# medvedevgroup/TwoPaCo

Measured on AMD Instinct MI355X. Metric: kmers_hashed_per_sec, higher is better.
Workload: dtype u64

## Files before the change

### twopaco_amd/csrc/tpc_capi.hip

```cpp
#include "tpc_ctx.h"

namespace tpch {

int fail(tpc_ctx *c, int code, const char *fmt, ...)
{
    char buf[512];
    va_list ap;
    va_start(ap, fmt);
    vsnprintf(buf, sizeof buf, fmt, ap);
    va_end(ap);
    if (c) c->err = buf;
    return code;
}





TpcLaunch make_launch(const tpc_ctx *c)
{
    TpcLaunch a;
    a.P = c->P; a.tab = c->tab; a.bases = c->bases; a.nmask = c->nmask; a.n_text = c->n_text;
    a.n_tiles = c->n_tiles; a.filter = c->filter; a.stream = c->stream;
    a.stat_kernel = c->stat_kernel;
// ... 175 lines not shown
bool replicated(const tpc_ctx *c) { return c->opt_replicate && c->sh_world > 1; }
void pass_tiles(const tpc_ctx *c, uint64_t &t_begin, uint64_t &t_end)
{
    const uint64_t tiles = text_tiles512(c);
    t_begin = 0; t_end = tiles;
    if (replicated(c)) {
        const uint64_t chunk = (tiles + c->sh_world - 1) / c->sh_world;
        t_begin = std::min<uint64_t>(tiles, (uint64_t)c->sh_rank * chunk);
        t_end = std::min<uint64_t>(tiles, t_begin + chunk);
    }
}
uint64_t pass_tile_count(const tpc_ctx *c) { uint64_t a, b; pass_tiles(c, a, b); return std::max<uint64_t>(1, b - a); }

size_t qpart_need(const TpcQPlan &pl, int i)
{
    if (i == 0) return std::max(tpc_qpart_bytes(pl, 0), tpc_qpart_bytes(pl, 9));
    if (i == 9) return 0;
    return tpc_qpart_bytes(pl, i);
}

bool part_hash_supported(const tpc_ctx *c)
{
    if (c->P.q > TPC_KERNEL_MAXQ || tpc_test_force_anyq) return false;
    if (c->P.q > 8 && (c->P.L - c->opt_slice_bits > 24 || c->no_lean)) return false;
    return true;
}

bool plan_query(const tpc_ctx *c, uint64_t lo, uint64_t hi, bool gated, TpcQPlan &pl)
{
    const uint64_t tiles = pass_tile_count(c);
    if (c->P.q > TPC_KERNEL_MAXQ || tpc_test_force_anyq) return false;
// ... 87 lines not shown
}

const char *tpc_last_error(const tpc_ctx *c) { return c ? c->err.c_str() : "null context"; }

int tpc_set_option(tpc_ctx *c, const char *name, int64_t value)
{
    if (!c || !name) return -1;
    if (!strcmp(name, "insert_test_first")) { c->opt_test_first = value != 0; return 0; }
    if (!strcmp(name, "insert_mode")) { c->opt_insert_mode = (int)value; return 0; }
    if (!strcmp(name, "slice_bits")) { c->opt_slice_bits = (int)value; return 0; }
    if (!strcmp(name, "query_mode")) { c->opt_query_mode = (int)value; return 0; }
    if (!strcmp(name, "part_budget_bytes")) { c->opt_part_budget = value; return 0; }
    if (!strcmp(name, "part_levels")) { c->opt_part_levels = (int)value; return 0; }
    if (!strcmp(name, "shard_tight_regions")) { c->opt_shard_tight = value ? 1 : 0; c->sh_have[0] = c->sh_have[1] = false; return 0; }
    if (!strcmp(name, "part_min_tiles")) { c->opt_part_min_tiles = value < 1 ? 1 : value; return 0; }
    if (!strcmp(name, "fuse_apply_lookup")) { c->opt_fuse = value != 0; return 0; }
    if (!strcmp(name, "test_q6_pb2")) { tpc_test_q6_pb2 = (int)value; return 0; }
    if (!strcmp(name, "insert_entry_fmt")) { tpc_test_insert_p3 = value == 3; return 0; }
    if (!strcmp(name, "shard_periodic_skip")) { c->opt_shard_periodic = value != 0; return 0; }
    if (!strcmp(name, "periodic_skip")) { c->opt_periodic = value != 0; if (!value) c->periodic_valid = false; return 0; }
    if (!strcmp(name, "test_tight_pinch")) { tpc_test_tight_pinch = (int)value; c->sh_have[0] = c->sh_have[1] = false; return 0; }
    if (!strcmp(name, "test_sched_cap")) { tpc_test_sched_cap = value > 0 ? (uint32_t)value : 0; return 0; }
    if (!strcmp(name, "text_window")) { c->opt_text_window = value != 0; return 0; }
    if (!strcmp(name, "replicate_filter")) { c->opt_replicate = value != 0; return 0; }
    if (!strcmp(name, "test_force_anyq")) { tpc_test_force_anyq = value != 0; return 0; }
    if (!strcmp(name, "test_sketch_grid")) { tpc_test_sketch_grid = value > 0 ? (int)value : 0; return 0; }
    if (!strcmp(name, "test_links_slots_log2")) { c->opt_links_slots_log2 = (int)std::max<int64_t>(-1, std::min<int64_t>(value, 64)); return 0; }
    if (!strcmp(name, "test_distances_chunk_words")) { c->opt_distances_chunk_words = (int)std::max<int64_t>(-1, std::min<int64_t>(value, 1 << 20)); return 0; }
    if (!strcmp(name, "test_fail_mallocs")) { tpc_test_fail_mallocs.store(value > 0 ? (int)value : 0); return 0; }
    return fail(c, -1, "unknown option %s", name);
// ... 17 lines not shown
{
    if (!c) return -1;
    return tpc_preload(c->device);
}

int64_t tpc_get_stat(const tpc_ctx *c, const char *name)
{
    if (!c || !name) return -1;
    if (!strcmp(name, "insert_path")) return c->stat_path[0];
    if (!strcmp(name, "query_path")) return c->stat_path[1];
    if (!strcmp(name, "insert_entry_fmt")) return c->stat_fmt[0];
    if (!strcmp(name, "query_entry_fmt")) return c->stat_fmt[1];
    if (!strcmp(name, "insert_hash_kernel")) return c->stat_kernel[0];
    if (!strcmp(name, "query_hash_kernel")) return c->stat_kernel[1];
    if (!strcmp(name, "query_verify_kernel")) return c->stat_kernel[2];
    if (!strcmp(name, "insert_batches")) return c->stat_batches[0];
    if (!strcmp(name, "query_batches")) return c->stat_batches[1];
    if (!strcmp(name, "query_tiles_per_batch")) return c->stat_q_plan[0];
    if (!strcmp(name, "query_b1")) return c->stat_q_plan[1];
    if (!strcmp(name, "query_b2")) return c->stat_q_plan[2];
    if (!strcmp(name, "query_begun")) return c->stat_q_begun;
    if (!strcmp(name, "filter2_retries")) return c->stat_filter2_retries;
    if (!strcmp(name, "aggregate_retries")) return c->stat_aggregate_retries;
    if (!strcmp(name, "filter2_counted")) return c->stat_filter2_counted;
    if (!strcmp(name, "fused_lookups")) return c->stat_fused;
    if (!strcmp(name, "query_overflow_entries")) return c->stat_query_overflow;
    if (!strcmp(name, "insert_overflow_entries")) return c->stat_insert_overflow;
    if (!strcmp(name, "periodic_skip")) return c->periodic_valid ? 1 : 0;
    if (!strcmp(name, "pbuf_releases")) return c->stat_pbuf_releases;
    if (!strcmp(name, "distances_tile")) return TPC_DISTANCES_TILE;
// ... 404 lines not shown
    if (part)
        for (int i = 0; i < tpc_ctx::NPBUF && part; i++) if (qpart_need(pl, i)) part = ensure_pbuf(c, i, qpart_need(pl, i));
    const bool fused = !begin_only && part && fuses(pl);
    if (!fused && !begin_only) { int rc0 = materialize_reset(c); if (rc0) return rc0; }
    if (part) {
        pl.buf1 = (uint64_t *)c->pbuf[0]; pl.cnt1 = (uint32_t *)c->pbuf[1]; pl.buf2 = (uint64_t *)c->pbuf[2]; pl.cnt2 = (uint32_t *)c->pbuf[3];
        pl.ovf = (uint64_t *)c->pbuf[4]; pl.ovf_cur = (unsigned long long *)c->pbuf[5];
        pl.surv = (uint64_t *)c->pbuf[6]; pl.surv_cur = (unsigned long long *)c->pbuf[7];
        pl.off2 = (const uint64_t *)c->pbuf[8];
        if (c->off2_uploaded != pl.off2_host) {
            HIPCHK(c, hipMemcpy(c->pbuf[8], pl.off2_host.data(), pl.off2_host.size() * 8, hipMemcpyHostToDevice));
            c->off2_uploaded = pl.off2_host;
        }
        pl.buf3 = (uint64_t *)c->pbuf[0]; pl.cnt3 = (uint32_t *)c->pbuf[10]; pl.off3 = (const uint64_t *)c->pbuf[11];
        pl.bnd = (uint32_t *)c->pbuf[18];
        if (pl.b3 && c->off3_uploaded != pl.off3_host) {
            HIPCHK(c, hipMemcpy(c->pbuf[11], pl.off3_host.data(), pl.off3_host.size() * 8, hipMemcpyHostToDevice));
            c->off3_uploaded = pl.off3_host;
        }
        unsigned long long f1[2] = {0, 0}, f2 = 0;
        bool overflowed = false;
        uint64_t per_batch = 1;
        {
            Timed t(c, TPC_K_QUERY);
            const uint64_t per = pl.n_tiles;
            per_batch = per;
            for (uint64_t t0 = t_begin; (t0 < t_end || t0 == t_begin) && !overflowed; t0 += per) {
                pl.tile0 = t0;
                pl.tile0_global = t0;
                pl.n_tiles = t0 < t_end ? std::min<uint64_t>(per, t_end - t0) : 0;
                const bool presplit = begun && t0 == t_begin;
                if (!presplit) {
                    HIPCHK(c, hipMemsetAsync(pl.ovf_cur, 0, 32 * sizeof(unsigned long long), c->stream));
                    HIPCHK(c, hipMemsetAsync(pl.surv_cur, 0, TPC_SURV_CUR_WORDS * sizeof(unsigned long long), c->stream));
                }
                if (begin_only) {
                    TpcQPlan p1 = pl;
                    p1.rbuf1 = p1.buf1; p1.rcnt1 = p1.cnt1;
                    if (tpc_launch_query_part_hash(make_launch_periodic(c), p1, c->rmask, lo, hi, gated) || tpc_launch_query_part_split(make_launch(c), p1))
                        return fail(c, -1, "partitioned query launch failed");
                    HIPCHK(c, hipGetLastError());
                    c->qb_valid = true; c->qb_lo = lo; c->qb_hi = hi;
// ... 22 lines not shown
                    p1.rbuf1 = p1.buf1; p1.rcnt1 = p1.cnt1;
                    p1.presplit = true;
                    if (tpc_launch_query_part_lookup(make_launch(c), p1) || tpc_launch_query_verify(make_launch(c), p1, c->rmask)) return fail(c, -1, "partitioned query launch failed");
                } else
                if (tpc_launch_query_partitioned(make_launch_periodic(c), pl, c->rmask, lo, hi, gated)) return fail(c, -1, "partitioned query launch failed");
                HIPCHK(c, hipMemcpyAsync(f1, pl.ovf_cur, sizeof f1, hipMemcpyDeviceToHost, c->stream));
                HIPCHK(c, hipMemcpyAsync(&f2, pl.surv_cur + 64, sizeof f2, hipMemcpyDeviceToHost, c->stream));
                if (t0 + per < t_end) {
                    unsigned long long sc[TPC_SURV_CUR_WORDS], batch_marks = 0;
                    const uint64_t w0 = t0 * 512, wn = std::min<uint64_t>(pl.n_tiles * 512, c->n_words > w0 ? c->n_words - w0 : 0);
                    if (wn) tpc_launch_mask_count(c->stream, c->rmask + w0, wn, c->block_sums, c->counters + 3);
                    HIPCHK(c, hipMemcpyAsync(sc, pl.surv_cur, sizeof sc, hipMemcpyDeviceToHost, c->stream));
                    if (wn) HIPCHK(c, hipMemcpyAsync(&batch_marks, c->counters + 3, sizeof batch_marks, hipMemcpyDeviceToHost, c->stream));
                    HIPCHK(c, hipStreamSynchronize(c->stream));
                    overflowed = f1[1] != 0 || f2 != 0;
                    unsigned long long surv = 0;
                    for (int i = 0; i < 64; i++) surv += std::min<unsigned long long>(sc[i], pl.surv_cap);
                    if (surv > 0) pl.group_survivors = batch_marks * 4 >= surv;
                }
            }
            if (c->periodic_valid && c->periodic_any_q && c->periodic) tpc_launch_periodic_copy(c->stream, c->rmask, c->periodic, c->periodic + c->n_words_alloc, c->n_words_alloc, c->n_words);
            tpc_launch_mask_count(c->stream, c->rmask, c->n_words, c->block_sums, c->counters + 1);
        }
        HIPCHK(c, hipGetLastError());
        uint64_t n = 0;
        int rc = read_counter(c, 1, &n);
        if (rc) return rc;
        overflowed = overflowed || f1[1] != 0 || f2 != 0;
        c->stat_query_overflow = (int64_t)f1[0];
        c->stat_path[1] = (pl.b3 ? 3 : 2) + (overflowed ? 10 : 0);
        c->stat_fmt[1] = pl.fmt;
        c->stat_batches[1] = (int64_t)((pass_tile_count(c) + per_batch - 1) / per_batch);
        c->stat_q_plan[0] = (int64_t)per_batch; c->stat_q_plan[1] = pl.b1; c->stat_q_plan[2] = pl.b2;
        if (c->dbg_ovf) {
            unsigned long long sc[65];
            (void)hipMemcpy(sc, pl.surv_cur, sizeof sc, hipMemcpyDeviceToHost);
            unsigned long long tot = 0, most = 0;
            for (int i = 0; i < 64; i++) { tot += sc[i]; most = std::max(most, sc[i]); }
            fprintf(stderr, "[ovf] query: %llu overflow entries (cap %llu, flag %llu), survivors %llu (fullest list %llu of %llu, flag %llu) b1=%d b2=%d ppr=%d loads=%d\n", f1[0],
                    (unsigned long long)pl.ovf_cap, f1[1], tot, most, (unsigned long long)pl.surv_cap, f2, pl.b1, pl.b2, pl.pos_per_round, pl.loads);
            static const char *const dump_path = getenv("TPC_DUMP_SURV");
            if (const char *path = dump_path) {
                if (FILE *fp = fopen(path, "w")) {
                    for (int i = 0; i < 64; i++) {
                        const size_t n = (size_t)std::min<unsigned long long>(sc[i], pl.surv_cap);
// ... 42 lines not shown
        }
        if (c->dbg_phases) {
            unsigned long long pr[32];
            (void)hipMemcpy(pr, pl.ovf_cur, sizeof pr, hipMemcpyDeviceToHost);
            fprintf(stderr, "[phases] ovf=%llu  split: push %llu book %llu copy %llu rounds %llu | hash: push %llu book %llu copy %llu rounds %llu (10 ns ticks summed over WGs) | lost at level 1: %llu, at level 2/3: %llu\n",
                    pr[0], pr[8], pr[9], pr[10], pr[12], pr[16], pr[17], pr[18], pr[20], pr[25], pr[27]);
        }
        if (!overflowed) {
            c->rmask_sums_valid = true;
            c->rmask_sums_n = n;
            if (n_marks) *n_marks = n;
            return 0;
        }
        if (replicated(c)) return fail(c, -20, "overflow or survivor list overflowed (address skew beyond what the sharded path handles)");
    }
    if (!part) { c->stat_path[1] = 1; c->stat_batches[1] = 1; }
    HIPCHK(c, hipMemsetAsync(c->counters + 1, 0, sizeof(unsigned long long), c->stream));
    {
        Timed t(c, TPC_K_QUERY);
        TpcLaunch ad = make_launch(c);
        if (replicated(c)) { ad.g_begin = t_begin * 512ull * TPC_RUN; ad.g_end = t_end * 512ull * TPC_RUN; }
        if (part) ad.stat_kernel = nullptr;
        if (tpc_launch_query(ad, c->rmask, lo, hi, gated, c->counters + 1)) return fail(c, -1, "query launch failed");
    }
    HIPCHK(c, hipGetLastError());
    uint64_t n = 0;
    int rc = read_counter(c, 1, &n);
    if (rc) return rc;
    if (n_marks) *n_marks = n;
    return 0;
}
// ... 83 lines not shown
```

### twopaco_amd/csrc/tpc_ctx.h

```cpp
#pragma once
#include "../../include/twopaco_hip.h"
#include "tpc_internal.h"

#include <algorithm>
#include <atomic>
#include <cmath>
#include <chrono>
#include <cstdarg>
#include <cstdio>
#include <cstdlib>
#include <cstring>
#include <string>
#include <vector>
#include <map>

struct tpc_ctx {
    int device = 0;
    hipStream_t stream = nullptr;
    std::string err;
    bool have_params = false;
    TpcHashParams P{};
    uint64_t tab_host[TPC_TAB_WORDS]{};
    uint64_t *tab = nullptr;
    int C = 1;
// ... 90 lines not shown
    int opt_slice_bits = 20;
    bool filter_zero_pending = false;
    static constexpr int NPBUF = 19;
    void *pbuf[NPBUF] = {};
    size_t pbytes[NPBUF] = {};
    std::vector<uint64_t> off2_uploaded, off3_uploaded;
    int opt_part_levels = 0;
    int opt_shard_tight = 1;
    int stat_path[2] = {0, 0};
    int64_t stat_batches[2] = {0, 0};
    mutable int stat_kernel[3] = {0, 0, 0};
    int stat_fmt[2] = {0, 0};
    int64_t stat_filter2_retries = 0;
    int64_t stat_aggregate_retries = 0;
    int stat_filter2_counted = 0;
    int64_t opt_part_min_tiles = 256;
    int64_t opt_part_budget = 0;
    int opt_query_mode = 0;
    int opt_fuse = 1;
    bool pending_apply = false;
    bool pending_fresh = false;
    bool pending_shard = false;
    TpcPartPlan pending_pl;
    void *ikeep[2] = {nullptr, nullptr};
    size_t ikeep_bytes[2] = {0, 0};
    uint64_t *ikeep_ovf = nullptr;
    uint64_t ikeep_ovf_cap = 0;
    uint64_t pending_novf = 0;
    uint32_t *iovf_cnt = nullptr;
    uint64_t *iovf_off = nullptr;
// ... 97 lines not shown
```

### twopaco_amd/csrc/tpc_internal.h

```cpp
#pragma once
#include "tpc_device.h"
#include <algorithm>
#include <cstdlib>
#include <vector>

struct TpcEnv {
    bool no_lean, rb_hash, verify_eager, gated_full;
    int ppr_insert, gated_loads, split_loads9;
    int slice_grid;
    static const TpcEnv &get()
    {
        static const TpcEnv e = [] {
            TpcEnv v;
            v.no_lean = getenv("TPC_NO_LEAN") != nullptr;
            v.rb_hash = getenv("TPC_RB_HASH") != nullptr;
            const char *lz = getenv("TPC_VERIFY_LAZY");
            v.verify_eager = lz && lz[0] == '0';
            v.gated_full = getenv("TPC_GATED_FULL_REGIONS") != nullptr;
            const char *p = getenv("TPC_PPR_INSERT"), *g = getenv("TPC_GATED_LOADS");
            v.ppr_insert = p ? atoi(p) : 0;
            v.gated_loads = g ? atoi(g) : 0;
            const char *s9 = getenv("TPC_SPLIT_LOADS9");
            v.split_loads9 = s9 ? atoi(s9) : 0;
            const char *lg = getenv("TPC_LOOKUP_GRID");
            int n_cu = 0, dev = 0;
            if (hipGetDevice(&dev) != hipSuccess || hipDeviceGetAttribute(&n_cu, hipDeviceAttributeMultiprocessorCount, dev) != hipSuccess || n_cu <= 0) { (void)hipGetLastError(); n_cu = 256; }
            v.slice_grid = lg ? atoi(lg) : 2 * n_cu;
            return v;
        }();
        return e;
    }
};

// ... 97 lines not shown
    uint64_t *ovf;
    unsigned long long *ovf_cur;
    uint64_t *surv;
    unsigned long long *surv_cur;
    uint32_t rank = 0, world = 1;
    const uint64_t *rbuf1 = nullptr;
    const uint32_t *rcnt1 = nullptr;
    const uint64_t *roff1 = nullptr;
    const uint64_t *rown1 = nullptr;
    const uint32_t *rowncnt1 = nullptr;
    bool group_survivors = true;
    int fmt = 0;
    bool presplit = false;
    uint32_t tiles_per_wg = 0, n_groups = 0, pb2 = 0;
    uint32_t *bnd = nullptr;
};
#define TPC_SURV_CUR_WORDS 72
bool tpc_qpart_plan(int L, int slice_bits, uint64_t n_tiles, double frac, TpcQPlan &pl, int levels = 0);
size_t tpc_qpart_bytes(const TpcQPlan &pl, int which);
bool tpc_qpart_plan_sharded(int L, int slice_bits, uint64_t n_tiles, double frac, uint32_t rank, uint32_t world, TpcQPlan &pl, int levels = 0, bool tight = false,
                            bool packed = false);
int tpc_launch_query_partitioned(const TpcLaunch &a, const TpcQPlan &pl, uint32_t *rmask, uint64_t lo, uint64_t hi, bool gated);
int tpc_launch_insert_part_split(const TpcLaunch &a, const TpcPartPlan &pl);
int tpc_launch_insert_part_apply_only(const TpcLaunch &a, const TpcPartPlan &pl, bool fresh);
struct TpcListSrc;
int tpc_launch_query_part_fused_lookup(const TpcLaunch &a, const TpcQPlan &pl, const TpcPartPlan &ipl, bool fresh, const uint64_t *iovf_sorted, const uint64_t *iovf_off,
                                       const TpcListSrc *lists = nullptr);
int tpc_launch_ovf_by_slice(const TpcLaunch &a, const uint64_t *list, uint64_t n, int slice_bits, uint32_t n_slices, uint32_t *cnt, uint32_t *cursor,
                            uint64_t *off, uint64_t *sorted, uint32_t rank = 0, uint32_t world = 1, int log_nb2 = 0);
#define TPC_FUSE_MAX_OVF (16ull << 20)
int tpc_launch_query_verify(const TpcLaunch &a, const TpcQPlan &pl, uint32_t *rmask);
extern int tpc_test_tight_pinch;
extern int tpc_test_q6_pb2;
extern int tpc_test_insert_p3;
extern uint32_t tpc_test_sched_cap;
int tpc_launch_region_offsets(const TpcLaunch &a, const uint32_t *cnt, uint32_t n_regions, uint64_t *off);
int tpc_launch_region_pack(const TpcLaunch &a, const void *regions, uint64_t cap_entries, uint32_t entry_bytes, const uint32_t *cnt, const uint64_t *off,
                           uint32_t n_regions, void *packed);
int tpc_launch_query_part_hash(const TpcLaunch &a, const TpcQPlan &pl, uint32_t *rmask, uint64_t lo, uint64_t hi, bool gated);
int tpc_launch_query_part_lookup(const TpcLaunch &a, const TpcQPlan &pl);
int tpc_launch_query_part_split(const TpcLaunch &a, const TpcQPlan &pl);
int tpc_launch_surv_gather(const TpcLaunch &a, const TpcQPlan &pl, uint64_t *out);
int tpc_launch_verify_addrs(const TpcLaunch &a, const TpcQPlan &pl, int fn, int fn_count, const uint64_t *sid, uint64_t n, uint64_t *addr_out, int32_t *owner_out,
                            unsigned long long *owner_counts = nullptr);
#define TPC_V_OWNER_SHIFT 56
int tpc_launch_finish(hipStream_t s, const TpcQPlan &pl, const uint64_t *sid, uint64_t n, int fn_count, const uint8_t *hit, const uint32_t *perm, uint32_t *rmask,
                      unsigned long long *n_marked);
// ... 103 lines not shown
```

### twopaco_amd/csrc/tpc_qpartition.hip

```cpp
#ifndef TPC_QPARTITION_PART
#define TPC_QPARTITION_PART 0
#endif
#include "tpc_rbins.h"
#include "tpc_bins3.h"
#include "tpc_binsp.h"
#include "tpc_lean.h"
#include "tpc_internal.h"
#include "tpc_lists.h"
#include <algorithm>
#include <type_traits>
#include <cstdio>
#include <cstdlib>
#include <cmath>

#if TPC_QPARTITION_PART == 0
int tpc_test_q6_pb2 = 0;
#endif

namespace {

constexpr int QE_E_SHIFT = 31;
constexpr uint64_t QE_REM_MASK = (1ull << QE_E_SHIFT) - 1ull;
constexpr int QS_LISTS = 64;

struct QOverflow {
    uint64_t *list;
    unsigned long long *cursor;
    uint64_t cap;
    __device__ __forceinline__ void push(uint64_t addr, uint64_t sid, int site = 0) const
    {
#ifdef TPC_PROFILE_PHASES
// ... 725 lines not shown
        if (hit) {
            const uint32_t lane = threadIdx.x & 63u, leader = (uint32_t)__ffsll((long long)m) - 1u;
            unsigned long long base = 0;
            if (lane == leader) base = atomicAdd(&surv_cur[0], (unsigned long long)__popcll(m));
            base = __shfl(base, (int)leader, 64);
            const unsigned long long o = base + (unsigned long long)__popcll(m & ((1ull << lane) - 1ull));
            if (o < surv_cap) surv[o] = list[2 * i + 1]; else surv_cur[QS_LISTS] = 1ull;
        }
    }
}

#endif
template <int Q>
__global__ void __launch_bounds__(256)
k_q_verify(TpcHashParams P, const uint64_t *__restrict__ tab, const uint64_t *__restrict__ bases, const uint32_t *__restrict__ filter,
           const uint64_t *__restrict__ surv, const unsigned long long *__restrict__ surv_cur, uint64_t surv_cap, uint64_t gbase, uint32_t *rmask)
{
    __shared__ uint64_t s_h[Q * 5], s_hk[Q * 5];
    if (threadIdx.x < Q * 5) { s_h[threadIdx.x] = tab[threadIdx.x]; s_hk[threadIdx.x] = tab[TPC_TAB_HK + threadIdx.x]; }
    __syncthreads();
    const int list = blockIdx.y;
    const uint64_t n = min((uint64_t)surv_cur[list], surv_cap);
    const uint64_t *my = surv + (uint64_t)list * surv_cap;
    const uint64_t stride = (uint64_t)gridDim.x * blockDim.x;
    for (uint64_t idx = (uint64_t)blockIdx.x * blockDim.x + threadIdx.x; idx < n; idx += stride) {
        const uint64_t sid = my[idx];
        if (sid == ~0ull) continue;
        const int e = (int)(sid & 7);
        const uint64_t g = gbase + (sid >> 3);
        const int c = e & 3;
        auto roll = [&](auto lo_tag, auto hi_tag, bool neg_strand, uint64_t (&h)[Q]) {
            constexpr int LO = decltype(lo_tag)::value, HI = decltype(hi_tag)::value;
#pragma unroll
            for (int i = LO; i < HI; i++) h[i] = 0;
            if (!neg_strand) {
                for (int t0 = 0; t0 < P.k; t0 += 32) {
                    uint64_t w = tpc_text_word(bases, g + t0);
                    const int m = min(32, P.k - t0);
                    for (int t = 0; t < m; t++) {
                        const int ch = (int)(w & 3);
                        w >>= 2;
#pragma unroll
// ... 39 lines not shown
#pragma unroll
                for (int i = 2; i < Q; i++) { addr[i] = edge(i, ng, hp[i]); wv[i] = filter[addr[i] >> 5]; }
#pragma unroll
                for (int i = 2; i < Q; i++) present = present && ((wv[i] >> ((uint32_t)addr[i] & 31u)) & 1u);
            }
        } else {
            roll(I1(), IQ(), false, hp);
            roll(I1(), IQ(), true, hn);
            uint64_t p[Q], nn[Q];
#pragma unroll
            for (int i = 0; i < Q; i++) { p[i] = edge(i, false, hp[i]); nn[i] = edge(i, true, hn[i]); }
            const bool ng = tpc_pick_neg<Q>(p, nn);
#pragma unroll
            for (int i = 1; i < Q; i++) present = present && probe(ng ? nn[i] : p[i]);
        }
        if (present) atomicOr(&rmask[g >> 5], 1u << ((uint32_t)g & 31u));
    }
}

template <int Q, bool LAZY>
__global__ void __launch_bounds__(256)
k_q_verify2(TpcHashParams P, const uint64_t *__restrict__ tab, const uint64_t *__restrict__ bases, const uint32_t *__restrict__ filter,
            const uint64_t *__restrict__ surv, const unsigned long long *__restrict__ surv_cur, uint64_t surv_cap, uint64_t gbase, uint32_t *rmask)
{
    extern __shared__ __attribute__((aligned(16))) unsigned char smem[];
    uint4 *s_t = reinterpret_cast<uint4 *>(smem);
    const int k = P.k, L = P.L;
    for (int i = threadIdx.x; i < (k + 1) * 4 * Q; i += 256) {
        const int t = i / (4 * Q), c = (i / Q) & 3, f = i % Q;
        const uint64_t a = q_rotl_n(tab[f * 5 + c], L, (k - t) % L), b = q_rotl_n(tab[f * 5 + 3 - c], L, t % L);
        s_t[i] = make_uint4((uint32_t)a, (uint32_t)(a >> 32), (uint32_t)b, (uint32_t)(b >> 32));
    }
    __syncthreads();
    const int list = blockIdx.y;
    const uint64_t n = min((uint64_t)surv_cur[list], surv_cap);
    const uint64_t *my = surv + (uint64_t)list * surv_cap;
    const uint64_t stride = (uint64_t)gridDim.x * blockDim.x;
    const uint64_t wmask = (1ull << (2 * k)) - 1ull;
    uint64_t idx = (uint64_t)blockIdx.x * blockDim.x + threadIdx.x;
    uint64_t sid_n = idx < n ? my[idx] : 0;
    uint64_t w_n = idx < n ? tpc_text_word_x2(bases, gbase + (sid_n == ~0ull ? 0ull : sid_n >> 3)) : 0;
    for (; idx < n; idx += stride) {
        const uint64_t sid = sid_n;
        const uint64_t w = w_n & wmask;
        if (idx + stride < n) {
            sid_n = my[idx + stride];
            w_n = tpc_text_word_x2(bases, gbase + (sid_n == ~0ull ? 0ull : sid_n >> 3));
        }
        if (sid == ~0ull) continue;
        const int e = (int)(sid & 7), c = e & 3;
        const uint64_t g = gbase + (sid >> 3);
        uint64_t E = e < 4 ? ((w << 2) | (uint64_t)c) : (w | ((uint64_t)c << (2 * k)));
        bool present = true;
        if constexpr (!LAZY || Q < 3) {
            uint64_t p[Q], nn[Q];
#pragma unroll
            for (int i = 0; i < Q; i++) { p[i] = 0; nn[i] = 0; }
            const uint4 *row = s_t;
            for (int t = 0; t <= k; t++) {
                const uint4 *r = row + ((uint32_t)E & 3u) * Q;
                E >>= 2;
                row += 4 * Q;
#pragma unroll
                for (int i = 0; i < Q; i++) {
// ... 66 lines not shown
                    e2 >>= 2;
                    row += 8 * Q;
#pragma unroll
                    for (int i = 2; i < Q; i++) {
                        const uint2 x = r[2 * i];
                        a[i] ^= ((uint64_t)x.y << 32) | x.x;
                    }
                }
                uint32_t wv[Q];
#pragma unroll
                for (int i = 2; i < Q; i++) wv[i] = filter[a[i] >> 5];
#pragma unroll
                for (int i = 2; i < Q; i++) present = present && ((wv[i] >> ((uint32_t)a[i] & 31u)) & 1u);
            }
        }
        if (present) atomicOr(&rmask[g >> 5], 1u << ((uint32_t)g & 31u));
    }
}

#if TPC_QPARTITION_PART == 0
#include "tpc_qpart6.h"
#endif

constexpr int RT_CHUNK = 4096, RT_MAXW = 64;
constexpr int V_OWNER_SHIFT = TPC_V_OWNER_SHIFT;
template <int Q>
__global__ void __launch_bounds__(256)
k_v_addrs(TpcHashParams P, const uint64_t *__restrict__ tab, const uint64_t *__restrict__ bases, const uint64_t *__restrict__ sid_list, uint64_t n,
          uint64_t gbase, PtPerm perm, PtShard sh, int log_nb2, int fn, int fn_count, uint64_t *__restrict__ addr_out, int32_t *__restrict__ owner_out,
          unsigned long long *owner_counts)
{
// ... 527 lines not shown
}

void launch_qsplit6(const TpcLaunch &a, const TpcQPlan &pl, QOverflow ovf)
{
    const PtShard sh{0, 1};
    const size_t lds_base = BinsP<PFmt6, QS_THREADS>::lds_bytes(pl.b2) + ((size_t)8 << pl.b2) + 64 + 128;
    uint32_t nreg_cap, sched_cap;
    size_t lds;
    pt_schedule_dims(pl.nwg1, pl.wpb, pl.cap1, (uint32_t)pl.loads * QS_THREADS, lds_base, nreg_cap, sched_cap, lds);
    (void)hipFuncSetAttribute((const void *)k_q_split<false, false, true>, hipFuncAttributeMaxDynamicSharedMemorySize, (int)lds);
    hipLaunchKernelGGL((k_q_split<false, false, true>), dim3((1u << pl.b1) * pl.wpb), dim3(QS_THREADS), lds, a.stream, pl.b1, pl.b2, a.P.L, pl.slice_bits, pl.loads, pl.nwg1, pl.wpb,
                       pl.rbuf1, pl.rcnt1, pl.cap1, pl.buf2, pl.cnt2, pl.off2, ovf, sh, 0u, 0, nreg_cap, sched_cap, pl.roff1, (const uint64_t *)nullptr, (const uint32_t *)nullptr,
                       pl.bnd, pl.n_groups, pl.tiles_per_wg, (uint32_t)pl.n_tiles, pl.pb2);
}

#endif
template <int Q>
void launch_qverify(const TpcLaunch &a, const TpcQPlan &pl, uint32_t *rmask)
{
    const uint64_t gbase = pl.tile0_global * (uint64_t)(PT_THREADS * TPC_RUN);
    const size_t table = (size_t)(a.P.k + 1) * 4 * Q * 16;
    if (a.P.k <= 31 && table <= 48 * 1024 && !TpcEnv::get().no_lean) {
        const bool lazy = !TpcEnv::get().verify_eager;
        if (a.stat_kernel) a.stat_kernel[2] = lazy ? 1 : 2;
        if (lazy) {
            (void)hipFuncSetAttribute((const void *)k_q_verify2<Q, true>, hipFuncAttributeMaxDynamicSharedMemorySize, (int)table);
            hipLaunchKernelGGL((k_q_verify2<Q, true>), dim3(256, QS_LISTS), dim3(256), table, a.stream, a.P, a.tab, a.bases, a.filter, pl.surv, pl.surv_cur, pl.surv_cap, gbase,
                               rmask);
        } else {
            (void)hipFuncSetAttribute((const void *)k_q_verify2<Q, false>, hipFuncAttributeMaxDynamicSharedMemorySize, (int)table);
            hipLaunchKernelGGL((k_q_verify2<Q, false>), dim3(256, QS_LISTS), dim3(256), table, a.stream, a.P, a.tab, a.bases, a.filter, pl.surv, pl.surv_cur, pl.surv_cap, gbase,
                               rmask);
        }
        return;
    }
    if (a.stat_kernel) a.stat_kernel[2] = 3;
    hipLaunchKernelGGL((k_q_verify<Q>), dim3(256, QS_LISTS), dim3(256), 0, a.stream, a.P, a.tab, a.bases, a.filter, pl.surv, pl.surv_cur, pl.surv_cap, gbase, rmask);
}

}

#if TPC_QPARTITION_PART == 0
bool tpc_qpart_plan(int L, int slice_bits, uint64_t n_tiles, double frac, TpcQPlan &pl, int levels)
{
    return tpc_qpart_plan_sharded(L, slice_bits, n_tiles, frac, 0, 1, pl, levels, false, true);
}

static bool qpart_plan_compute(int L, int slice_bits, uint64_t n_tiles, double frac, uint32_t rank, uint32_t world, TpcQPlan &pl, int levels, bool tight, bool packed);

bool tpc_qpart_plan_sharded(int L, int slice_bits, uint64_t n_tiles, double frac, uint32_t rank, uint32_t world, TpcQPlan &pl, int levels, bool tight, bool packed)
{
    struct Key { int L, slice_bits, levels, q6; uint64_t n_tiles; double frac; uint32_t rank, world; bool tight, packed; };
    static thread_local Key last{};
    static thread_local TpcQPlan last_pl;
    static thread_local bool have = false, last_ok = false;
    const Key k{L, slice_bits, levels, tpc_test_q6_pb2 + (tpc_test_tight_pinch << 8), n_tiles, frac, rank, world, tight, packed};
    if (have && k.L == last.L && k.slice_bits == last.slice_bits && k.levels == last.levels && k.q6 == last.q6 && k.n_tiles == last.n_tiles && k.frac == last.frac &&
        k.rank == last.rank && k.world == last.world && k.tight == last.tight && k.packed == last.packed) {
        if (last_ok) pl = last_pl;
        return last_ok;
    }
    last_ok = qpart_plan_compute(L, slice_bits, n_tiles, frac, rank, world, pl, levels, tight, packed);
    last = k; have = true;
    if (last_ok) last_pl = pl;
    return last_ok;
}

static bool qpart_plan_compute(int L, int slice_bits, uint64_t n_tiles, double frac, uint32_t rank, uint32_t world, TpcQPlan &pl, int levels, bool tight, bool packed)
{
    pl = TpcQPlan();
    pl.rank = rank; pl.world = world;
    const uint64_t n_text = n_tiles * PT_THREADS * TPC_RUN;
    const int F = L - slice_bits;
    if (F < 2 || slice_bits < 6 || slice_bits > 20) return false;
    if (n_text > (1ull << 30)) return false;
    pl.slice_bits = slice_bits;
    const bool three = levels == 3 || (levels == 0 && F > 18);
    if (three) {
        if (F < 3) return false;
        pl.b1 = std::max((F + 2) / 3, L - 31);
// ... 118 lines not shown
        }
    }
    switch (which) {
    case 0: return (size_t)pl.nwg1 * (1u << pl.b1) * pl.cap1 * 8;
    case 1: return (size_t)pl.nwg1 * (1u << pl.b1) * 4;
    case 2: return (size_t)pl.buf2_entries * 8;
    case 3: return ((size_t)((1u << pl.b1) / pl.world) * pl.wpb * (1u << pl.b2)) * 4;
    case 4: return pl.ovf_cap * 16;
    case 5: return 32 * sizeof(unsigned long long);
    case 6: return (size_t)QS_LISTS * pl.surv_cap * 8;
    case 7: return TPC_SURV_CUR_WORDS * sizeof(unsigned long long);
    case 8: return pl.off2_host.size() * 8;
    case 9: return (size_t)pl.buf3_entries * 8;
    case 10: return pl.b3 ? (((size_t)pl.wpb3 << (pl.b1 + pl.b2 + pl.b3)) / pl.world) * 4 : 0;
    case 11: return pl.off3_host.size() * 8;
    }
    return 0;
}

int tpc_launch_query_part_hash(const TpcLaunch &a, const TpcQPlan &pl, uint32_t *rmask, uint64_t lo, uint64_t hi, bool gated)
{
    if (a.P.q < 1 || a.P.q > TPC_KERNEL_MAXQ) return -1;
    launch_qhash(a, pl, gated, lo, hi, rmask);
    return 0;
}

int tpc_launch_query_part_split(const TpcLaunch &a, const TpcQPlan &pl)
{
    const PtShard sh{pl.rank, pl.world};
    QOverflow ovf{pl.ovf, pl.ovf_cur, pl.ovf_cap};
// ... 91 lines not shown
        (void)hipFuncSetAttribute((const void *)k_apply_lookup, hipFuncAttributeMaxDynamicSharedMemorySize, (int)lds);
        if (a.ev_lookup0) (void)hipEventRecord(a.ev_lookup0, a.stream);
        hipLaunchKernelGGL(k_apply_lookup, dim3(ls.n_src ? (1u << (pl.b1 + pl.b2)) / pl.world : tpc_slice_grid((1u << (pl.b1 + pl.b2)) / pl.world)), dim3(PT_APPLY_THREADS), lds, a.stream, pl.slice_bits, pl.b2, ipl.wpb, ipl.buf2, ipl.cnt2,
                           ipl.cap2, fresh ? 1 : 0, iovf, iovf_off, pl.wpb, pl.buf2, pl.cnt2, pl.off2, a.filter, pl.surv, pl.surv_cur, pl.surv_cap, perm, pl.group_survivors ? 1 : 0, sh, ls, (uint32_t)((1u << (pl.b1 + pl.b2)) / pl.world));
        if (a.ev_lookup1) (void)hipEventRecord(a.ev_lookup1, a.stream);
    }
    hipLaunchKernelGGL(k_q_ovf, dim3(1024), dim3(256), 0, a.stream, pl.ovf, pl.ovf_cur, pl.ovf_cap, a.filter, pl.surv, pl.surv_cur, pl.surv_cap, perm, sh, pl.b2);
    return 0;
}

#endif
int tpc_launch_query_verify_other(const TpcLaunch &a, const TpcQPlan &pl, uint32_t *rmask);
#if TPC_QPARTITION_PART == 0
int tpc_launch_query_verify(const TpcLaunch &a, const TpcQPlan &pl, uint32_t *rmask)
{
    if (a.P.q == 5) { launch_qverify<5>(a, pl, rmask); return 0; }
    return tpc_launch_query_verify_other(a, pl, rmask);
}

int tpc_launch_query_partitioned(const TpcLaunch &a, const TpcQPlan &pl0, uint32_t *rmask, uint64_t lo, uint64_t hi, bool gated)
{
    TpcQPlan pl = pl0;
    pl.rbuf1 = pl.buf1;
    pl.rcnt1 = pl.cnt1;
    int rc = tpc_launch_query_part_hash(a, pl, rmask, lo, hi, gated);
    if (rc) return rc;
    if ((rc = tpc_launch_query_part_lookup(a, pl))) return rc;
    return tpc_launch_query_verify(a, pl, rmask);
}
#else
int tpc_launch_query_verify_other(const TpcLaunch &a, const TpcQPlan &pl, uint32_t *rmask)
{
// ... 153 lines not shown
```

Before: 12.27 billion.

## Route verify hits through binned mark lists instead of global atomicOr

The verify kernels now write each survivor's pass/fail position into a compact pass array instead of issuing scattered global atomicOr on the result mask. Two new kernels follow. One bins passing positions by region into per-workgroup buckets. The other applies each region's marks to an LDS copy of the mask slice and writes it back. This is meant to replace random global atomics with LDS atomics and coalesced writes, at the cost of two extra kernel launches, extra buffer space and a fallback atomic path when a bucket overflows. It is enabled by default through opt_verify_marks and can be overridden by an environment variable.

Measured after the change: 12.54 billion (median of 6 runs). +2.2%, better.

```diff
diff --git a/twopaco_amd/csrc/tpc_capi.hip b/twopaco_amd/csrc/tpc_capi.hip
--- a/twopaco_amd/csrc/tpc_capi.hip
+++ b/twopaco_amd/csrc/tpc_capi.hip
@@ -213,7 +213,7 @@
 
 size_t qpart_need(const TpcQPlan &pl, int i)
 {
-    if (i == 0) return std::max(tpc_qpart_bytes(pl, 0), tpc_qpart_bytes(pl, 9));
+    if (i == 0) return std::max({tpc_qpart_bytes(pl, 0), tpc_qpart_bytes(pl, 9), tpc_qpart_bytes(pl, 19)});
     if (i == 9) return 0;
     return tpc_qpart_bytes(pl, i);
 }
@@ -331,6 +331,10 @@
     if (!strcmp(name, "part_levels")) { c->opt_part_levels = (int)value; return 0; }
     if (!strcmp(name, "shard_tight_regions")) { c->opt_shard_tight = value ? 1 : 0; c->sh_have[0] = c->sh_have[1] = false; return 0; }
     if (!strcmp(name, "part_min_tiles")) { c->opt_part_min_tiles = value < 1 ? 1 : value; return 0; }
+    if (!strcmp(name, "verify_marks")) { c->opt_verify_marks = value != 0; return 0; }
+    if (!strcmp(name, "mark_bucket_bits")) { tpc_test_mark_bucket_bits = (int)value; return 0; }
+    if (!strcmp(name, "mark_region_cap")) { tpc_test_mark_region_cap = (int)value; return 0; }
+    if (!strcmp(name, "mark_slice_bits")) { tpc_test_mark_slice_bits = (int)value; return 0; }
     if (!strcmp(name, "fuse_apply_lookup")) { c->opt_fuse = value != 0; return 0; }
     if (!strcmp(name, "test_q6_pb2")) { tpc_test_q6_pb2 = (int)value; return 0; }
     if (!strcmp(name, "insert_entry_fmt")) { tpc_test_insert_p3 = value == 3; return 0; }
@@ -378,6 +382,8 @@
     if (!strcmp(name, "insert_hash_kernel")) return c->stat_kernel[0];
     if (!strcmp(name, "query_hash_kernel")) return c->stat_kernel[1];
     if (!strcmp(name, "query_verify_kernel")) return c->stat_kernel[2];
+    if (!strcmp(name, "query_mark_path")) return c->stat_mark_path;
+    if (!strcmp(name, "query_mark_fallback")) return c->stat_mark_fallback;
     if (!strcmp(name, "insert_batches")) return c->stat_batches[0];
     if (!strcmp(name, "query_batches")) return c->stat_batches[1];
     if (!strcmp(name, "query_tiles_per_batch")) return c->stat_q_plan[0];
@@ -812,18 +818,23 @@
         }
         pl.buf3 = (uint64_t *)c->pbuf[0]; pl.cnt3 = (uint32_t *)c->pbuf[10]; pl.off3 = (const uint64_t *)c->pbuf[11];
         pl.bnd = (uint32_t *)c->pbuf[18];
+        pl.pass = pl.mark_buf = pl.mark_cnt = nullptr;
+        const int env_marks = TpcEnv::get().verify_marks;
+        const bool mark_lists = env_marks >= 0 ? env_marks != 0 : c->opt_verify_marks != 0;
+        if (mark_lists && tpc_qpart_bytes(pl, 19) <= c->pbytes[0]) tpc_qpart_mark_pointers(pl, c->pbuf[0]);
         if (pl.b3 && c->off3_uploaded != pl.off3_host) {
             HIPCHK(c, hipMemcpy(c->pbuf[11], pl.off3_host.data(), pl.off3_host.size() * 8, hipMemcpyHostToDevice));
             c->off3_uploaded = pl.off3_host;
         }
-        unsigned long long f1[2] = {0, 0}, f2 = 0;
-        bool overflowed = false;
+        unsigned long long f1[3] = {0, 0, 0}, f2 = 0, lost_marks = 0;
+        bool overflowed = false, f1_counted = false;
         uint64_t per_batch = 1;
         {
             Timed t(c, TPC_K_QUERY);
             const uint64_t per = pl.n_tiles;
             per_batch = per;
             for (uint64_t t0 = t_begin; (t0 < t_end || t0 == t_begin) && !overflowed; t0 += per) {
+                f1_counted = false;
                 pl.tile0 = t0;
                 pl.tile0_global = t0;
                 pl.n_tiles = t0 < t_end ? std::min<uint64_t>(per, t_end - t0) : 0;
@@ -876,6 +887,8 @@
                     if (wn) HIPCHK(c, hipMemcpyAsync(&batch_marks, c->counters + 3, sizeof batch_marks, hipMemcpyDeviceToHost, c->stream));
                     HIPCHK(c, hipStreamSynchronize(c->stream));
                     overflowed = f1[1] != 0 || f2 != 0;
+                    lost_marks += f1[2];
+                    f1_counted = true;
                     unsigned long long surv = 0;
                     for (int i = 0; i < 64; i++) surv += std::min<unsigned long long>(sc[i], pl.surv_cap);
                     if (surv > 0) pl.group_survivors = batch_marks * 4 >= surv;
@@ -889,8 +902,11 @@
         int rc = read_counter(c, 1, &n);
         if (rc) return rc;
         overflowed = overflowed || f1[1] != 0 || f2 != 0;
+        if (!f1_counted) lost_marks += f1[2];
         c->stat_query_overflow = (int64_t)f1[0];
         c->stat_path[1] = (pl.b3 ? 3 : 2) + (overflowed ? 10 : 0);
+        c->stat_mark_path = pl.pass && !overflowed ? 1 : 0;
+        c->stat_mark_fallback = c->stat_mark_path ? (int64_t)lost_marks : 0;
         c->stat_fmt[1] = pl.fmt;
         c->stat_batches[1] = (int64_t)((pass_tile_count(c) + per_batch - 1) / per_batch);
         c->stat_q_plan[0] = (int64_t)per_batch; c->stat_q_plan[1] = pl.b1; c->stat_q_plan[2] = pl.b2;
@@ -963,7 +979,7 @@
         }
         if (replicated(c)) return fail(c, -20, "overflow or survivor list overflowed (address skew beyond what the sharded path handles)");
     }
-    if (!part) { c->stat_path[1] = 1; c->stat_batches[1] = 1; }
+    if (!part) { c->stat_path[1] = 1; c->stat_batches[1] = 1; c->stat_mark_path = 0; c->stat_mark_fallback = 0; }
     HIPCHK(c, hipMemsetAsync(c->counters + 1, 0, sizeof(unsigned long long), c->stream));
     {
         Timed t(c, TPC_K_QUERY);
diff --git a/twopaco_amd/csrc/tpc_ctx.h b/twopaco_amd/csrc/tpc_ctx.h
--- a/twopaco_amd/csrc/tpc_ctx.h
+++ b/twopaco_amd/csrc/tpc_ctx.h
@@ -128,6 +128,9 @@
     int64_t stat_filter2_retries = 0;
     int64_t stat_aggregate_retries = 0;
     int stat_filter2_counted = 0;
+    int opt_verify_marks = 1;
+    int stat_mark_path = 0;
+    int64_t stat_mark_fallback = 0;
     int64_t opt_part_min_tiles = 256;
     int64_t opt_part_budget = 0;
     int opt_query_mode = 0;
diff --git a/twopaco_amd/csrc/tpc_internal.h b/twopaco_amd/csrc/tpc_internal.h
--- a/twopaco_amd/csrc/tpc_internal.h
+++ b/twopaco_amd/csrc/tpc_internal.h
@@ -6,6 +6,7 @@
 
 struct TpcEnv {
     bool no_lean, rb_hash, verify_eager, gated_full;
+    int verify_marks;
     int ppr_insert, gated_loads, split_loads9;
     int slice_grid;
     static const TpcEnv &get()
@@ -17,6 +18,8 @@
             const char *lz = getenv("TPC_VERIFY_LAZY");
             v.verify_eager = lz && lz[0] == '0';
             v.gated_full = getenv("TPC_GATED_FULL_REGIONS") != nullptr;
+            const char *vm = getenv("TPC_VERIFY_MARKS");
+            v.verify_marks = vm && vm[0] ? (vm[0] != '0' ? 1 : 0) : -1;
             const char *p = getenv("TPC_PPR_INSERT"), *g = getenv("TPC_GATED_LOADS");
             v.ppr_insert = p ? atoi(p) : 0;
             v.gated_loads = g ? atoi(g) : 0;
@@ -144,10 +147,16 @@
     bool presplit = false;
     uint32_t tiles_per_wg = 0, n_groups = 0, pb2 = 0;
     uint32_t *bnd = nullptr;
+    uint32_t *pass = nullptr;
+    uint32_t *mark_buf = nullptr;
+    uint32_t *mark_cnt = nullptr;
+    int MB = 0, mark_lnb = 0, mark_sub_bits = 0;
+    uint32_t mark_nb = 0, mark_wg = 0, mark_cap = 0;
 };
 #define TPC_SURV_CUR_WORDS 72
 bool tpc_qpart_plan(int L, int slice_bits, uint64_t n_tiles, double frac, TpcQPlan &pl, int levels = 0);
 size_t tpc_qpart_bytes(const TpcQPlan &pl, int which);
+void tpc_qpart_mark_pointers(TpcQPlan &pl, void *base);
 bool tpc_qpart_plan_sharded(int L, int slice_bits, uint64_t n_tiles, double frac, uint32_t rank, uint32_t world, TpcQPlan &pl, int levels = 0, bool tight = false,
                             bool packed = false);
 int tpc_launch_query_partitioned(const TpcLaunch &a, const TpcQPlan &pl, uint32_t *rmask, uint64_t lo, uint64_t hi, bool gated);
@@ -161,6 +170,7 @@
 #define TPC_FUSE_MAX_OVF (16ull << 20)
 int tpc_launch_query_verify(const TpcLaunch &a, const TpcQPlan &pl, uint32_t *rmask);
 extern int tpc_test_tight_pinch;
+extern int tpc_test_mark_bucket_bits, tpc_test_mark_region_cap, tpc_test_mark_slice_bits;
 extern int tpc_test_q6_pb2;
 extern int tpc_test_insert_p3;
 extern uint32_t tpc_test_sched_cap;
diff --git a/twopaco_amd/csrc/tpc_qpartition.hip b/twopaco_amd/csrc/tpc_qpartition.hip
--- a/twopaco_amd/csrc/tpc_qpartition.hip
+++ b/twopaco_amd/csrc/tpc_qpartition.hip
@@ -15,6 +15,7 @@
 
 #if TPC_QPARTITION_PART == 0
 int tpc_test_q6_pb2 = 0;
+int tpc_test_mark_bucket_bits = 0, tpc_test_mark_region_cap = 0, tpc_test_mark_slice_bits = 0;
 #endif
 
 namespace {
@@ -770,7 +771,7 @@
 template <int Q>
 __global__ void __launch_bounds__(256)
 k_q_verify(TpcHashParams P, const uint64_t *__restrict__ tab, const uint64_t *__restrict__ bases, const uint32_t *__restrict__ filter,
-           const uint64_t *__restrict__ surv, const unsigned long long *__restrict__ surv_cur, uint64_t surv_cap, uint64_t gbase, uint32_t *rmask)
+           const uint64_t *__restrict__ surv, const unsigned long long *__restrict__ surv_cur, uint64_t surv_cap, uint64_t gbase, uint32_t *rmask, uint32_t *__restrict__ pass)
 {
     __shared__ uint64_t s_h[Q * 5], s_hk[Q * 5];
     if (threadIdx.x < Q * 5) { s_h[threadIdx.x] = tab[threadIdx.x]; s_hk[threadIdx.x] = tab[TPC_TAB_HK + threadIdx.x]; }
@@ -778,10 +779,14 @@
     const int list = blockIdx.y;
     const uint64_t n = min((uint64_t)surv_cur[list], surv_cap);
     const uint64_t *my = surv + (uint64_t)list * surv_cap;
+    uint32_t *my_pass = pass ? pass + (uint64_t)list * surv_cap : nullptr;
     const uint64_t stride = (uint64_t)gridDim.x * blockDim.x;
     for (uint64_t idx = (uint64_t)blockIdx.x * blockDim.x + threadIdx.x; idx < n; idx += stride) {
         const uint64_t sid = my[idx];
-        if (sid == ~0ull) continue;
+        if (sid == ~0ull) {
+            if (my_pass) my_pass[idx] = 0xFFFFFFFFu;
+            continue;
+        }
         const int e = (int)(sid & 7);
         const uint64_t g = gbase + (sid >> 3);
         const int c = e & 3;
@@ -851,14 +856,15 @@
 #pragma unroll
             for (int i = 1; i < Q; i++) present = present && probe(ng ? nn[i] : p[i]);
         }
-        if (present) atomicOr(&rmask[g >> 5], 1u << ((uint32_t)g & 31u));
+        if (my_pass) my_pass[idx] = present ? (uint32_t)(sid >> 3) : 0xFFFFFFFFu;
+        else if (present) atomicOr(&rmask[g >> 5], 1u << ((uint32_t)g & 31u));
     }
 }
 
 template <int Q, bool LAZY>
 __global__ void __launch_bounds__(256)
 k_q_verify2(TpcHashParams P, const uint64_t *__restrict__ tab, const uint64_t *__restrict__ bases, const uint32_t *__restrict__ filter,
-            const uint64_t *__restrict__ surv, const unsigned long long *__restrict__ surv_cur, uint64_t surv_cap, uint64_t gbase, uint32_t *rmask)
+            const uint64_t *__restrict__ surv, const unsigned long long *__restrict__ surv_cur, uint64_t surv_cap, uint64_t gbase, uint32_t *rmask, uint32_t *__restrict__ pass)
 {
     extern __shared__ __attribute__((aligned(16))) unsigned char smem[];
     uint4 *s_t = reinterpret_cast<uint4 *>(smem);
@@ -872,6 +878,7 @@
     const int list = blockIdx.y;
     const uint64_t n = min((uint64_t)surv_cur[list], surv_cap);
     const uint64_t *my = surv + (uint64_t)list * surv_cap;
+    uint32_t *my_pass = pass ? pass + (uint64_t)list * surv_cap : nullptr;
     const uint64_t stride = (uint64_t)gridDim.x * blockDim.x;
     const uint64_t wmask = (1ull << (2 * k)) - 1ull;
     uint64_t idx = (uint64_t)blockIdx.x * blockDim.x + threadIdx.x;
@@ -884,7 +891,10 @@
             sid_n = my[idx + stride];
             w_n = tpc_text_word_x2(bases, gbase + (sid_n == ~0ull ? 0ull : sid_n >> 3));
         }
-        if (sid == ~0ull) continue;
+        if (sid == ~0ull) {
+            if (my_pass) my_pass[idx] = 0xFFFFFFFFu;
+            continue;
+        }
         const int e = (int)(sid & 7), c = e & 3;
         const uint64_t g = gbase + (sid >> 3);
         uint64_t E = e < 4 ? ((w << 2) | (uint64_t)c) : (w | ((uint64_t)c << (2 * k)));
@@ -981,7 +991,8 @@
                 for (int i = 2; i < Q; i++) present = present && ((wv[i] >> ((uint32_t)a[i] & 31u)) & 1u);
             }
         }
-        if (present) atomicOr(&rmask[g >> 5], 1u << ((uint32_t)g & 31u));
+        if (my_pass) my_pass[idx] = present ? (uint32_t)(sid >> 3) : 0xFFFFFFFFu;
+        else if (present) atomicOr(&rmask[g >> 5], 1u << ((uint32_t)g & 31u));
     }
 }
 
@@ -1539,6 +1550,134 @@
                        pl.bnd, pl.n_groups, pl.tiles_per_wg, (uint32_t)pl.n_tiles, pl.pb2);
 }
 
+constexpr int MK_LOADS = 4;
+__global__ void __launch_bounds__(1024)
+k_mark_split(const uint32_t *__restrict__ pass, const unsigned long long *__restrict__ surv_cur, uint64_t surv_cap, int MB, int LOG_NB, uint32_t nb, uint32_t *mark_buf,
+             uint32_t *mark_cnt, uint32_t cap, uint64_t gbase, uint32_t *rmask, unsigned long long *n_lost)
+{
+    extern __shared__ __attribute__((aligned(16))) unsigned char smem[];
+    Bins3<uint32_t, 1024> bins;
+    (void)bins.carve(smem, LOG_NB);
+    const uint32_t wg = blockIdx.x, per = gridDim.x / QS_LISTS;
+    bins.init(mark_buf, [=](uint32_t b) { return b < nb ? make_uint2((uint32_t)((((uint64_t)wg * nb + b) * cap) >> 5), cap) : make_uint2(0u, 0u); });
+    auto lost = [=](uint32_t b, uint32_t val) {
+        const uint64_t g = gbase + ((uint64_t)b << MB) + val;
+        atomicOr(&rmask[g >> 5], 1u << ((uint32_t)g & 31u));
+        atomicAdd(n_lost, 1ull);
+    };
+    __syncthreads();
+    const uint32_t list = wg / per, part = wg % per;
+    const uint64_t n = min((uint64_t)surv_cur[list], surv_cap);
+    const uint64_t chunk = ((n + per - 1) / per + 3) & ~3ull;
+    const uint64_t begin = min(n, (uint64_t)part * chunk), end = min(n, begin + chunk);
+    const uint32_t *src = pass + (uint64_t)list * surv_cap;
+    const uint32_t low = (1u << MB) - 1u;
+    constexpr uint64_t STEP = (uint64_t)MK_LOADS * 1024;
+    if (begin < end) {
+        uint32_t va[MK_LOADS], vb[MK_LOADS];
+        auto load = [&](uint32_t (&d)[MK_LOADS], uint64_t base) {
+#pragma unroll
+            for (int i = 0; i < MK_LOADS; i++) d[i] = src[min(base + (uint64_t)i * 1024 + threadIdx.x, end - 1)];
+        };
+        auto round = [&](const uint32_t (&cur)[MK_LOADS], uint64_t base) {
+            uint32_t bb[MK_LOADS], val[MK_LOADS];
+            bool ok[MK_LOADS];
+#pragma unroll
+            for (int i = 0; i < MK_LOADS; i++) {
+                ok[i] = base + (uint64_t)i * 1024 + threadIdx.x < end && cur[i] != 0xFFFFFFFFu;
+                bb[i] = ok[i] ? cur[i] >> MB : 0u;
+                val[i] = cur[i] & low;
+            }
+            bins.template push_batch<MK_LOADS>(bb, val, ok, lost);
+            bins.template flush<false>(lost);
+        };
+        load(va, begin);
+        for (uint64_t base = begin;; base += 2 * STEP) {
+            if (base + STEP < end) load(vb, base + STEP);
+            round(va, base);
+            if (base + STEP >= end) break;
+            if (base + 2 * STEP < end) load(va, base + 2 * STEP);
+            round(vb, base + STEP);
+            if (base + 2 * STEP >= end) break;
+        }
+    }
+    bins.template flush<true>(lost);
+    bins.store_counts(mark_cnt + ((uint64_t)wg << LOG_NB), [](uint32_t b) { return b; });
+}
+
+__global__ void __launch_bounds__(PT_APPLY_THREADS)
+k_mark_apply(int MB, int sub_bits, int LOG_NB, uint32_t nb, uint32_t nwg, const uint32_t *__restrict__ mark_buf, const uint32_t *__restrict__ mark_cnt, uint32_t cap,
+             uint64_t word_base, uint64_t n_words, uint32_t *rmask, uint32_t n_units)
+{
+    extern __shared__ __attribute__((aligned(16))) unsigned char smem[];
+    uint32_t *slice = reinterpret_cast<uint32_t *>(smem);
+    const uint32_t words = 1u << (sub_bits - 5), sub_log = (uint32_t)(MB - sub_bits), sub_mask = (1u << sub_bits) - 1u;
+    uint32_t *s_off = slice + words;
+    uint32_t *s_w = s_off + nwg + 1;
+    for (uint32_t u = blockIdx.x; u < n_units; u += gridDim.x) {
+        const uint32_t b = u >> sub_log, sub = u & ((1u << sub_log) - 1u);
+        const uint64_t w0 = word_base + ((uint64_t)b << (MB - 5)) + ((uint64_t)sub << (sub_bits - 5));
+        const uint32_t nw = w0 < n_words ? (uint32_t)min((uint64_t)words, n_words - w0) : 0u;
+        for (uint32_t i = threadIdx.x; i < words; i += PT_APPLY_THREADS) slice[i] = i < nw ? rmask[w0 + i] : 0u;
+        uint32_t running = 0;
+        for (uint32_t r0 = 0; r0 < nwg; r0 += PT_APPLY_THREADS) {
+            const uint32_t r = r0 + threadIdx.x;
+            const uint32_t n4 = r < nwg ? (min(mark_cnt[((uint64_t)r << LOG_NB) + b], cap) + 3u) >> 2 : 0u;
+            uint32_t total;
+            const uint32_t off = running + pt_block_excl_scan<PT_APPLY_THREADS>(n4, s_w, total);
+            if (r < nwg) s_off[r] = off;
+            running += total;
+            pt_barrier_lds();
+        }
+        if (threadIdx.x == 0) s_off[nwg] = running;
+        __syncthreads();
+        const uint32_t total4 = running;
+        constexpr int UNR = 4;
+        for (uint32_t i0 = threadIdx.x; i0 < total4; i0 += UNR * PT_APPLY_THREADS) {
+            uint4 v[UNR];
+#pragma unroll
+            for (int k = 0; k < UNR; k++) {
+                const uint32_t i = i0 + (uint32_t)k * PT_APPLY_THREADS;
+                v[k] = make_uint4(~0u, ~0u, ~0u, ~0u);
+                if (i < total4) {
+                    uint32_t lo = 0, hi = nwg;
+                    while (hi - lo > 1u) {
+                        const uint32_t mid = (lo + hi) >> 1;
+                        if (s_off[mid] <= i) lo = mid; else hi = mid;
+                    }
+                    v[k] = reinterpret_cast<const uint4 *>(mark_buf + ((uint64_t)lo * nb + b) * cap)[i - s_off[lo]];
+                }
+            }
+#pragma unroll
+            for (int k = 0; k < UNR; k++) {
+                const uint32_t e[4] = {v[k].x, v[k].y, v[k].z, v[k].w};
+#pragma unroll
+                for (int j = 0; j < 4; j++)
+                    if (e[j] != 0xFFFFFFFFu && (e[j] >> sub_bits) == sub) atomicOr(&slice[(e[j] & sub_mask) >> 5], 1u << (e[j] & 31u));
+            }
+        }
+        __syncthreads();
+        for (uint32_t i = threadIdx.x; i < nw; i += PT_APPLY_THREADS) rmask[w0 + i] = slice[i];
+        __syncthreads();
+    }
+}
+
+void launch_marks(const TpcLaunch &a, const TpcQPlan &pl, uint32_t *rmask)
+{
+    const uint64_t gbase = pl.tile0_global * (uint64_t)(PT_THREADS * TPC_RUN);
+    const size_t lds_split = Bins3<uint32_t, 1024>::lds_bytes(pl.mark_lnb);
+    (void)hipFuncSetAttribute((const void *)k_mark_split, hipFuncAttributeMaxDynamicSharedMemorySize, (int)lds_split);
+    hipLaunchKernelGGL(k_mark_split, dim3(pl.mark_wg), dim3(1024), lds_split, a.stream, pl.pass, pl.surv_cur, pl.surv_cap, pl.MB, pl.mark_lnb, pl.mark_nb, pl.mark_buf, pl.mark_cnt,
+                       pl.mark_cap, gbase, rmask, pl.ovf_cur + 2);
+    const uint64_t n_pos = std::max<uint64_t>(1, pl.n_tiles) * (uint64_t)(PT_THREADS * TPC_RUN);
+    const uint32_t nb_used = (uint32_t)std::min<uint64_t>(pl.mark_nb, (n_pos + (1ull << pl.MB) - 1) >> pl.MB);
+    const uint32_t n_units = nb_used << (pl.MB - pl.mark_sub_bits);
+    const size_t lds_apply = ((size_t)4 << (pl.mark_sub_bits - 5)) + ((size_t)pl.mark_wg + 1 + 16) * 4;
+    (void)hipFuncSetAttribute((const void *)k_mark_apply, hipFuncAttributeMaxDynamicSharedMemorySize, (int)lds_apply);
+    hipLaunchKernelGGL(k_mark_apply, dim3(tpc_slice_grid(n_units)), dim3(PT_APPLY_THREADS), lds_apply, a.stream, pl.MB, pl.mark_sub_bits, pl.mark_lnb, pl.mark_nb, pl.mark_wg, pl.mark_buf,
+                       pl.mark_cnt, pl.mark_cap, gbase >> 5, (a.n_text >> 5) + 1, rmask, n_units);
+}
+
 #endif
 template <int Q>
 void launch_qverify(const TpcLaunch &a, const TpcQPlan &pl, uint32_t *rmask)
@@ -1551,16 +1690,16 @@
         if (lazy) {
             (void)hipFuncSetAttribute((const void *)k_q_verify2<Q, true>, hipFuncAttributeMaxDynamicSharedMemorySize, (int)table);
             hipLaunchKernelGGL((k_q_verify2<Q, true>), dim3(256, QS_LISTS), dim3(256), table, a.stream, a.P, a.tab, a.bases, a.filter, pl.surv, pl.surv_cur, pl.surv_cap, gbase,
-                               rmask);
+                               rmask, pl.pass);
         } else {
             (void)hipFuncSetAttribute((const void *)k_q_verify2<Q, false>, hipFuncAttributeMaxDynamicSharedMemorySize, (int)table);
             hipLaunchKernelGGL((k_q_verify2<Q, false>), dim3(256, QS_LISTS), dim3(256), table, a.stream, a.P, a.tab, a.bases, a.filter, pl.surv, pl.surv_cur, pl.surv_cap, gbase,
-                               rmask);
+                               rmask, pl.pass);
         }
         return;
     }
     if (a.stat_kernel) a.stat_kernel[2] = 3;
-    hipLaunchKernelGGL((k_q_verify<Q>), dim3(256, QS_LISTS), dim3(256), 0, a.stream, a.P, a.tab, a.bases, a.filter, pl.surv, pl.surv_cur, pl.surv_cap, gbase, rmask);
+    hipLaunchKernelGGL((k_q_verify<Q>), dim3(256, QS_LISTS), dim3(256), 0, a.stream, a.P, a.tab, a.bases, a.filter, pl.surv, pl.surv_cur, pl.surv_cap, gbase, rmask, pl.pass);
 }
 
 }
@@ -1572,6 +1711,7 @@
 }
 
 static bool qpart_plan_compute(int L, int slice_bits, uint64_t n_tiles, double frac, uint32_t rank, uint32_t world, TpcQPlan &pl, int levels, bool tight, bool packed);
+static void qpart_plan_marks(TpcQPlan &pl);
 
 bool tpc_qpart_plan_sharded(int L, int slice_bits, uint64_t n_tiles, double frac, uint32_t rank, uint32_t world, TpcQPlan &pl, int levels, bool tight, bool packed)
 {
@@ -1582,13 +1722,44 @@
     const Key k{L, slice_bits, levels, tpc_test_q6_pb2 + (tpc_test_tight_pinch << 8), n_tiles, frac, rank, world, tight, packed};
     if (have && k.L == last.L && k.slice_bits == last.slice_bits && k.levels == last.levels && k.q6 == last.q6 && k.n_tiles == last.n_tiles && k.frac == last.frac &&
         k.rank == last.rank && k.world == last.world && k.tight == last.tight && k.packed == last.packed) {
-        if (last_ok) pl = last_pl;
+        if (last_ok) { pl = last_pl; qpart_plan_marks(pl); }
         return last_ok;
     }
     last_ok = qpart_plan_compute(L, slice_bits, n_tiles, frac, rank, world, pl, levels, tight, packed);
     last = k; have = true;
-    if (last_ok) last_pl = pl;
+    if (last_ok) { last_pl = pl; qpart_plan_marks(pl); }
     return last_ok;
+}
+
+static void qpart_plan_marks(TpcQPlan &pl)
+{
+    const uint64_t n_text = std::max<uint64_t>(1, pl.n_tiles) * PT_THREADS * TPC_RUN;
+    int MB = 14;
+    while (((n_text + (1ull << MB) - 1) >> MB) > 512) ++MB;
+    const int tb = tpc_test_mark_bucket_bits;
+    if (tb >= 14 && tb <= 21 && ((n_text + (1ull << tb) - 1) >> tb) <= 512) MB = tb;
+    pl.MB = MB;
+    pl.mark_nb = (uint32_t)((n_text + (1ull << MB) - 1) >> MB);
+    pl.mark_lnb = 4;
+    while ((1u << pl.mark_lnb) < pl.mark_nb) ++pl.mark_lnb;
+    int sub = std::min(MB, 20);
+    if (tpc_test_mark_slice_bits >= 10 && tpc_test_mark_slice_bits < sub) sub = tpc_test_mark_slice_bits;
+    pl.mark_sub_bits = sub;
+    pl.mark_wg = QS_LISTS * (n_text >= (1ull << 24) ? 4u : 1u);
+    const double mean = (double)QS_LISTS * (double)pl.surv_cap / ((double)pl.mark_wg * (double)pl.mark_nb);
+    pl.mark_cap = (uint32_t)(((uint64_t)(mean * 1.3 + 8 * std::sqrt(mean) + 32) + 31) & ~31ull);
+    if (tpc_test_mark_region_cap > 0) pl.mark_cap = (uint32_t)((std::min(tpc_test_mark_region_cap, 1 << 20) + 31) & ~31);
+}
+
+static size_t mark_pass_bytes(const TpcQPlan &pl) { return (((size_t)QS_LISTS * pl.surv_cap * 4) + 127) & ~(size_t)127; }
+static size_t mark_buf_bytes(const TpcQPlan &pl) { return (size_t)pl.mark_wg * pl.mark_nb * pl.mark_cap * 4; }
+
+void tpc_qpart_mark_pointers(TpcQPlan &pl, void *base)
+{
+    unsigned char *p = static_cast<unsigned char *>(base);
+    pl.pass = reinterpret_cast<uint32_t *>(p);
+    pl.mark_buf = reinterpret_cast<uint32_t *>(p + mark_pass_bytes(pl));
+    pl.mark_cnt = reinterpret_cast<uint32_t *>(p + mark_pass_bytes(pl) + mark_buf_bytes(pl));
 }
 
 static bool qpart_plan_compute(int L, int slice_bits, uint64_t n_tiles, double frac, uint32_t rank, uint32_t world, TpcQPlan &pl, int levels, bool tight, bool packed)
@@ -1737,6 +1908,7 @@
     case 9: return (size_t)pl.buf3_entries * 8;
     case 10: return pl.b3 ? (((size_t)pl.wpb3 << (pl.b1 + pl.b2 + pl.b3)) / pl.world) * 4 : 0;
     case 11: return pl.off3_host.size() * 8;
+    case 19: return mark_pass_bytes(pl) + mark_buf_bytes(pl) + ((size_t)pl.mark_wg << pl.mark_lnb) * 4;
     }
     return 0;
 }
@@ -1858,8 +2030,10 @@
 #if TPC_QPARTITION_PART == 0
 int tpc_launch_query_verify(const TpcLaunch &a, const TpcQPlan &pl, uint32_t *rmask)
 {
-    if (a.P.q == 5) { launch_qverify<5>(a, pl, rmask); return 0; }
-    return tpc_launch_query_verify_other(a, pl, rmask);
+    if (a.P.q == 5) launch_qverify<5>(a, pl, rmask);
+    else if (int rc = tpc_launch_query_verify_other(a, pl, rmask)) return rc;
+    if (pl.pass) launch_marks(a, pl, rmask);
+    return 0;
 }
 
 int tpc_launch_query_partitioned(const TpcLaunch &a, const TpcQPlan &pl0, uint32_t *rmask, uint64_t lo, uint64_t hi, bool gated)
```
